# bryanlimy/CalciumGAN

Measured on AMD Instinct MI355X. Metric: training samples/sec (seq_len=2048, n_critic=5), higher is better.
Workload: dtype bf16; 1 GPU; cfg2: dichotomised-Gaussian sl2048 calcium signals, 102 neurons, batch 128/GPU, calciumgan num_units 64 k 24 s 2 m 10 layer_norm, wgan-gp n_critic 5 lambda 10, Keras Adam 1e-4; global_batch=128, seq_len=2048, parallelism=dp1, launch=hipGraph replay of train(), critic_layer1_on_interpolate=a*y_real + (1-a)*y_fake from the stored outputs (cg_lrelu_mix)

## Files before the change

### calciumgan_amd/csrc/dense_rows.hip

```cpp
#include "cg_common.h"

namespace {

constexpr int kDrThreads = 256;
constexpr int kDrPitch = 132;

struct DenseRowsArgs {
  const uint16_t* x;
  const uint16_t* w;
  const float* bias;
  float* y;
  long long rows;
  int Cx, N, Cy, epilogue;
};

template <int KSTEPS>
__global__ __launch_bounds__(kDrThreads, 2) void dense_rows_kernel(
    DenseRowsArgs a) {
  __shared__ float tile[4][16 * kDrPitch];
  const int lane = threadIdx.x & 63;
  const int wave = threadIdx.x >> 6;
  const int r16 = lane & 15;
  const int g = lane >> 4;
  act8 wf[KSTEPS][8];
// ... 1 lines not shown
  for (int ks = 0; ks < KSTEPS; ++ks)
#pragma unroll
    for (int nt = 0; nt < 8; ++nt)
      wf[ks][nt] = *reinterpret_cast<const act8*>(
          a.w + (((long long)(nt * 16 + r16) * KSTEPS + ks) * 16 + g) * 8);
  float* tl = tile[wave];
  const int tcol = (lane & 31) * 4;
  const int trow = lane >> 5;
  f32x4 bv = {0.f, 0.f, 0.f, 0.f};
  f32x4 keep = {0.f, 0.f, 0.f, 0.f};
#pragma unroll
  for (int e = 0; e < 4; ++e)
    if (tcol + e < a.N) {
      keep[e] = 1.f;
      if (a.bias) bv[e] = a.bias[tcol + e];
    }
  const bool sig = a.epilogue == CG_EPI_SIGMOID;

  const long long nblk = (a.rows + 15) / 16;
  const long long stride = (long long)gridDim.x * 4;
  long long blk = (long long)blockIdx.x * 4 + wave;
  auto load_a = [&](long long b, act8 (&dst)[KSTEPS]) {
    const long long row = b * 16 + r16;
    const bool ok = b < nblk && row < a.rows;
#pragma unroll
    for (int ks = 0; ks < KSTEPS; ++ks) {
      act8 v = {0, 0, 0, 0, 0, 0, 0, 0};
      if (ok)
        v = *reinterpret_cast<const act8*>(a.x + row * a.Cx + ks * 32 + g * 8);
      dst[ks] = v;
    }
  };
  auto compute = [&](long long b, const act8 (&af)[KSTEPS]) {
    f32x4 acc[8];
#pragma unroll
    for (int nt = 0; nt < 8; ++nt) acc[nt] = f32x4{0.f, 0.f, 0.f, 0.f};
#pragma unroll
    for (int ks = 0; ks < KSTEPS; ++ks)
#pragma unroll
      for (int nt = 0; nt < 8; ++nt)
        acc[nt] = cg_mfma_16x16x32(af[ks], wf[ks][nt],
                                                          acc[nt], 0, 0, 0);
#pragma unroll
    for (int nt = 0; nt < 8; ++nt)
#pragma unroll
      for (int r = 0; r < 4; ++r)
        tl[(4 * g + r) * kDrPitch + nt * 16 + r16] = acc[nt][r];
    __builtin_amdgcn_fence(__ATOMIC_RELEASE, "wavefront");
    __builtin_amdgcn_wave_barrier();
    __builtin_amdgcn_fence(__ATOMIC_ACQUIRE, "wavefront");
#pragma unroll 2
    for (int pass = 0; pass < 8; ++pass) {
      const int row = pass * 2 + trow;
      const long long m = b * 16 + row;
      f32x4 v = *reinterpret_cast<const f32x4*>(tl + row * kDrPitch + tcol);
#pragma unroll
      for (int e = 0; e < 4; ++e) {
        const float t = v[e] + bv[e];
        const float sg = 1.f / (1.f + __expf(-t));
        v[e] = keep[e] != 0.f ? (sig ? sg : t) : 0.f;
      }
      if (m < a.rows && tcol < a.Cy)
        *reinterpret_cast<f32x4*>(a.y + m * a.Cy + tcol) = v;
    }
    __builtin_amdgcn_fence(__ATOMIC_RELEASE, "wavefront");
    __builtin_amdgcn_wave_barrier();
    __builtin_amdgcn_fence(__ATOMIC_ACQUIRE, "wavefront");
  };
  act8 af0[KSTEPS], af1[KSTEPS];
  load_a(blk, af0);
  while (blk < nblk) {
    load_a(blk + stride, af1);
    compute(blk, af0);
    blk += stride;
    if (blk >= nblk) break;
    load_a(blk + stride, af0);
    compute(blk, af1);
    blk += stride;
  }
}


constexpr int kMaxInterp = 8;
struct DenseInterpArgs {
  const uint16_t* x;
  const uint16_t* w;
  const float* bias;
  const float* real;
  const float* alpha;
  uint16_t* x0[kMaxInterp];
  int n, B, L, Cx, N, Cr, Cp, epilogue;
};

template <int KSTEPS>
__global__ __launch_bounds__(kDrThreads, 2) void dense_rows_interp_kernel(
    DenseInterpArgs a) {
  __shared__ float tile[4][16 * kDrPitch];
  const int lane = threadIdx.x & 63;
  const int wave = threadIdx.x >> 6;
  const int r16 = lane & 15;
  const int g = lane >> 4;
  act8 wf[KSTEPS][8];
#pragma unroll
  for (int ks = 0; ks < KSTEPS; ++ks)
#pragma unroll
    for (int nt = 0; nt < 8; ++nt)
      wf[ks][nt] = *reinterpret_cast<const act8*>(
          a.w + (((long long)(nt * 16 + r16) * KSTEPS + ks) * 16 + g) * 8);
  float* tl = tile[wave];
  const int tcol = (lane & 31) * 4;
  const int trow = lane >> 5;
  f32x4 bv = {0.f, 0.f, 0.f, 0.f};
  f32x4 keep = {0.f, 0.f, 0.f, 0.f};
#pragma unroll
  for (int e = 0; e < 4; ++e)
    if (tcol + e < a.N) {
      keep[e] = 1.f;
      if (a.bias) bv[e] = a.bias[tcol + e];
    }
  const bool sig = a.epilogue == CG_EPI_SIGMOID;
  const long long R = (long long)a.B * a.L;
  const long long nblk = R / 16;
  const long long nitem = nblk * a.n;
  const long long stride = (long long)gridDim.x * 4;
  const long long seg = R * a.Cp;
  auto load_a = [&](long long blk, int k, bool ok, act8 (&dst)[KSTEPS]) {
    const long long row = (long long)k * R + blk * 16 + r16;
#pragma unroll
    for (int ks = 0; ks < KSTEPS; ++ks) {
      act8 v = {0, 0, 0, 0, 0, 0, 0, 0};
      if (ok) v = *reinterpret_cast<const act8*>(a.x + row * a.Cx + ks * 32 + g * 8);
      dst[ks] = v;
    }
  };
  auto store4 = [&](uint16_t* p, const f32x4& v) {
    *reinterpret_cast<uint2*>(p) = make_uint2(pack2act(v[0], v[1]), pack2act(v[2], v[3]));
  };
  auto compute = [&](long long blk, int k, const act8 (&af)[KSTEPS]) {
    f32x4 acc[8];
#pragma unroll
    for (int nt = 0; nt < 8; ++nt) acc[nt] = f32x4{0.f, 0.f, 0.f, 0.f};
#pragma unroll
    for (int ks = 0; ks < KSTEPS; ++ks)
#pragma unroll
      for (int nt = 0; nt < 8; ++nt)
        acc[nt] = cg_mfma_16x16x32(af[ks], wf[ks][nt], acc[nt], 0, 0, 0);
#pragma unroll
    for (int nt = 0; nt < 8; ++nt)
#pragma unroll
      for (int r = 0; r < 4; ++r)
        tl[(4 * g + r) * kDrPitch + nt * 16 + r16] = acc[nt][r];
    f32x4 rr[8];
#pragma unroll
    for (int pass = 0; pass < 8; ++pass) {
      const long long m = blk * 16 + pass * 2 + trow;
      const float* p = a.real + m * a.Cr + tcol;
      f32x4 v = {0.f, 0.f, 0.f, 0.f};
#pragma unroll
      for (int e = 0; e < 4; ++e)
        if (tcol + e < a.N) v[e] = p[e];
      rr[pass] = v;
    }
    __builtin_amdgcn_fence(__ATOMIC_RELEASE, "wavefront");
    __builtin_amdgcn_wave_barrier();
    __builtin_amdgcn_fence(__ATOMIC_ACQUIRE, "wavefront");
    const int b = (int)((blk * 16) / a.L);
    const float al = a.alpha ? a.alpha[k * a.B + b] : 0.f;
    uint16_t* x0 = a.x0[k];
#pragma unroll 2
    for (int pass = 0; pass < 8; ++pass) {
      const int row = pass * 2 + trow;
      const long long m = blk * 16 + row;
      f32x4 f = *reinterpret_cast<const f32x4*>(tl + row * kDrPitch + tcol);
      f32x4 xh;
#pragma unroll
      for (int e = 0; e < 4; ++e) {
        const float t = f[e] + bv[e];
        const float sg = 1.f / (1.f + __expf(-t));
        f[e] = keep[e] != 0.f ? (sig ? sg : t) : 0.f;
        xh[e] = al * rr[pass][e] + (1.f - al) * f[e];
      }
      if (tcol < a.Cp) {
        uint16_t* q = x0 + m * a.Cp + tcol;
        store4(q, rr[pass]);
        store4(q + seg, f);
        if (a.alpha) store4(q + 2 * seg, xh);
      }
    }
    __builtin_amdgcn_fence(__ATOMIC_RELEASE, "wavefront");
    __builtin_amdgcn_wave_barrier();
    __builtin_amdgcn_fence(__ATOMIC_ACQUIRE, "wavefront");
  };
  long long blk = (long long)blockIdx.x * 4 + wave;
  int k = 0;
  auto advance = [&](long long& bb, int& kk) {
    if (++kk == a.n) { kk = 0; bb += stride; }
  };
  act8 af0[KSTEPS], af1[KSTEPS];
  load_a(blk, k, blk < nblk, af0);
  (void)nitem;
  while (blk < nblk) {
    long long nb = blk; int nk = k;
    advance(nb, nk);
    load_a(nb, nk, nb < nblk, af1);
    compute(blk, k, af0);
    blk = nb; k = nk;
    if (blk >= nblk) break;
    advance(nb, nk);
    load_a(nb, nk, nb < nblk, af0);
    compute(blk, k, af1);
    blk = nb; k = nk;
  }
}

constexpr int kWideThreads = 256;
constexpr int kWideCols = 128;

struct DenseWideArgs {
  const uint16_t* x;
  const uint16_t* w;
  const float* bias;
  void* y;
  long long rows;
  int Cx, N, Cy, epilogue, out_act, panels;
  const float* real;
  const float* alpha;
  uint16_t* x0[kMaxInterp];
  long long seg_rows;
  int n_upd, L, Cr;
};

template <int KSTEPS>
__global__ __launch_bounds__(kWideThreads, KSTEPS <= 4 ? 2 : 1) void dense_rows_wide_kernel(
    DenseWideArgs a) {
  constexpr int kRowB = KSTEPS * 64 + 16;
  extern __shared__ __attribute__((aligned(16))) unsigned char wl[];
  const int tid = threadIdx.x;
  const int lane = tid & 63;
  const int wave = tid >> 6;
  const int r16 = lane & 15;
  const int g = lane >> 4;
  const int xcd = blockIdx.x & 7;
  const int j = blockIdx.x >> 3;
  const int panel = j % a.panels;
  const int rgroup = (j / a.panels) * 8 + xcd;
  const int ngroups = (int)(gridDim.x / 8 / a.panels) * 8;
  const int n0 = panel * kWideCols;
  for (int i = tid; i < kWideCols * KSTEPS * 4; i += kWideThreads) {
    const int c = i / (KSTEPS * 4);
    const int ks = (i / 4) % KSTEPS;
    const int gg = i & 3;
    const uint4 v = *reinterpret_cast<const uint4*>(
        a.w + (((long long)(n0 + c) * KSTEPS + ks) * 16 + gg) * 8);
    *reinterpret_cast<uint4*>(wl + c * kRowB + (ks * 4 + gg) * 16) = v;
  }
  __syncthreads();
  const int cq = (g & 1) * 16 + (g >> 1) * 8;
  float bv[4][8];
#pragma unroll
  for (int p = 0; p < 4; ++p)
#pragma unroll
    for (int e = 0; e < 8; ++e) {
      const int n = n0 + p * 32 + cq + e;
      bv[p][e] = (a.bias && n < a.N) ? a.bias[n] : 0.f;
    }
  const bool sig = a.epilogue == CG_EPI_SIGMOID;
  const int woff0 = r16 * kRowB + g * 16;

  const long long nblk = (a.rows + 31) / 32;
  const long long stride = (long long)ngroups * 4;
  long long blk = (long long)rgroup * 4 + wave;
  auto load_x = [&](long long b, act8 (&dst)[2][KSTEPS]) {
#pragma unroll
    for (int h = 0; h < 2; ++h) {
      long long row = b * 32 + h * 16 + r16;
      row = row < a.rows ? row : a.rows - 1;
      const uint16_t* src = a.x + row * a.Cx + g * 8;
#pragma unroll
      for (int ks = 0; ks < KSTEPS; ++ks)
        dst[h][ks] = *reinterpret_cast<const act8*>(src + ks * 32);
    }
  };
  auto compute = [&](long long b, const act8 (&xf)[2][KSTEPS]) {
    f32x4 acc[2][8];
#pragma unroll
    for (int h = 0; h < 2; ++h)
#pragma unroll
      for (int nt = 0; nt < 8; ++nt) acc[h][nt] = f32x4{0.f, 0.f, 0.f, 0.f};
    int woff = woff0;
    asm volatile("" : "+v"(woff));
    const unsigned char* wrow = wl + woff;
    act8 wa[8], wb[8];
// ... 31 lines not shown
    }
#pragma unroll
    for (int h = 0; h < 2; ++h) {
      const long long m = b * 32 + h * 16 + r16;
#pragma unroll
      for (int p = 0; p < 4; ++p) {
        float v[8];
#pragma unroll
        for (int r = 0; r < 4; ++r) {
          const auto sw = __builtin_amdgcn_permlane16_swap(
              __float_as_uint(acc[h][2 * p][r]),
              __float_as_uint(acc[h][2 * p + 1][r]), false, false);
          v[r] = __uint_as_float(sw[0]);
          v[4 + r] = __uint_as_float(sw[1]);
        }
        const int n = n0 + p * 32 + cq;
        if (m < a.rows && n < a.Cy) {
#pragma unroll
          for (int e = 0; e < 8; ++e) {
            const float t = v[e] + bv[p][e];
            const float sg = 1.f / (1.f + __expf(-t));
            v[e] = (n + e < a.N) ? (sig ? sg : t) : 0.f;
          }
          if (interp) {
            const long long rem = m - kupd * a.seg_rows;
            uint16_t* q = x0k + rem * a.Cy + n;
            const long long seg = a.seg_rows * a.Cy;
            *reinterpret_cast<uint4*>(q + seg) =
                make_uint4(pack2act(v[0], v[1]), pack2act(v[2], v[3]),
                           pack2act(v[4], v[5]), pack2act(v[6], v[7]));
            if (a.real) {
              const float* rp = a.real + rem * a.Cr + n;
              float rv[8], xh[8];
#pragma unroll
              for (int e = 0; e < 8; ++e) rv[e] = (n + e < a.N) ? rp[e] : 0.f;
              *reinterpret_cast<uint4*>(q) =
                  make_uint4(pack2act(rv[0], rv[1]), pack2act(rv[2], rv[3]),
                             pack2act(rv[4], rv[5]), pack2act(rv[6], rv[7]));
              if (a.alpha) {
                const float al =
                    a.alpha[kupd * (a.seg_rows / a.L) + (int)(rem / a.L)];
#pragma unroll
                for (int e = 0; e < 8; ++e) xh[e] = al * rv[e] + (1.f - al) * v[e];
                *reinterpret_cast<uint4*>(q + 2 * seg) =
                    make_uint4(pack2act(xh[0], xh[1]), pack2act(xh[2], xh[3]),
                               pack2act(xh[4], xh[5]), pack2act(xh[6], xh[7]));
              }
            }
          } else if (a.out_act) {
            *reinterpret_cast<uint4*>(reinterpret_cast<uint16_t*>(a.y) +
                                      m * a.Cy + n) =
                make_uint4(pack2act(v[0], v[1]), pack2act(v[2], v[3]),
                           pack2act(v[4], v[5]), pack2act(v[6], v[7]));
          } else {
            float* dst = reinterpret_cast<float*>(a.y) + m * a.Cy + n;
            *reinterpret_cast<f32x4*>(dst) = f32x4{v[0], v[1], v[2], v[3]};
            *reinterpret_cast<f32x4*>(dst + 4) = f32x4{v[4], v[5], v[6], v[7]};
          }
        }
      }
    }
  };
  act8 xf0[2][KSTEPS], xf1[2][KSTEPS];
  load_x(blk, xf0);
  while (blk < nblk) {
    load_x(blk + stride, xf1);
    compute(blk, xf0);
    blk += stride;
    if (blk >= nblk) break;
    load_x(blk + stride, xf0);
    compute(blk, xf1);
    blk += stride;
  }
}

template <int KSTEPS>
int launch_dense_wide(const DenseWideArgs& a, hipStream_t s) {
  const size_t lds = (size_t)kWideCols * (KSTEPS * 64 + 16);
  if (int e = cg_allow_dynamic_lds<&dense_rows_wide_kernel<KSTEPS>>(160 * 1024))
    return e;
  const int per_xcd = (KSTEPS <= 4 ? 64 : 32) / a.panels * a.panels;
  hipLaunchKernelGGL(dense_rows_wide_kernel<KSTEPS>, dim3(8 * per_xcd),
                     dim3(kWideThreads), lds, s, a);
  CG_LAUNCH_CHECK();
}

struct DenseWideInterp {
  const float* real;
  const float* alpha;
  void* const* x0;
  int n, B, L, Cr;
};

int dense_rows_wide(const void* x, const void* w, const float* bias, void* y,
                    long long rows, int Cx, int N, int Cy, int epilogue,
                    int out_act, hipStream_t s,
                    const DenseWideInterp* ip = nullptr) {
  if (Cx % 32 || N < 1 || Cy < N || Cy % 8) return CG_EINVAL;
  DenseWideArgs a;
  a.x = reinterpret_cast<const uint16_t*>(x);
  a.w = reinterpret_cast<const uint16_t*>(w);
  a.bias = bias;
  a.y = y;
  a.rows = rows;
  a.Cx = Cx; a.N = N; a.Cy = Cy; a.epilogue = epilogue; a.out_act = out_act;
  a.real = nullptr; a.alpha = nullptr; a.seg_rows = 1; a.n_upd = 0; a.L = 1; a.Cr = 0;
  for (int k = 0; k < kMaxInterp; ++k) a.x0[k] = nullptr;
  if (ip) {
    const long long seg = (long long)ip->B * ip->L;
    if (!ip->x0 || ip->n < 1 || ip->n > kMaxInterp || seg % 32 ||
        rows != seg * ip->n || (ip->real && ip->Cr < N) || (!ip->real && ip->alpha))
      return CG_EINVAL;
    a.real = ip->real; a.alpha = ip->alpha; a.seg_rows = seg;
    a.n_upd = ip->n; a.L = ip->L; a.Cr = ip->Cr;
    for (int k = 0; k < ip->n; ++k) {
      a.x0[k] = reinterpret_cast<uint16_t*>(ip->x0[k]);
      if (!a.x0[k]) return CG_EINVAL;
    }
  }
  a.panels = (N + kWideCols - 1) / kWideCols;
  if (a.panels > 32) return CG_EINVAL;
  switch (Cx / 32) {
    case 4: return launch_dense_wide<4>(a, s);
    case 8: return launch_dense_wide<8>(a, s);
    case 12: return launch_dense_wide<12>(a, s);
    case 16: return launch_dense_wide<16>(a, s);
    default: return CG_EINVAL;
  }
}

constexpr int kDwThreads = 256;
constexpr int kDwPitch = 144;

struct DenseWgradArgs {
  const uint16_t* x;
  const uint16_t* g;
  float* dw;
  long long rows, rows_per_split;
  int Cx, Cg, Cx_real, Cg_real, tiles_x, tiles_g;
  float* part;
};

__device__ __forceinline__ s16x4 dw_tr_read(const uint16_t* p) {
  return __builtin_amdgcn_ds_read_tr16_b64_v4i16(
      (__attribute__((address_space(3))) s16x4*)(p));
}
__device__ __forceinline__ act8 dw_join(s16x4 lo, s16x4 hi) {
  typedef __attribute__((ext_vector_type(8))) short s16x8;
  s16x8 v = {lo[0], lo[1], lo[2], lo[3], hi[0], hi[1], hi[2], hi[3]};
  return __builtin_bit_cast(act8, v);
}

__global__ __launch_bounds__(kDwThreads, 2) void dense_wgrad_kernel(
    DenseWgradArgs a) {
  __shared__ __attribute__((aligned(16))) uint16_t lx[2][32 * kDwPitch];
  __shared__ __attribute__((aligned(16))) uint16_t lg[2][32 * kDwPitch];
  const int tid = threadIdx.x;
  const int lane = tid & 63;
  const int wave = tid >> 6;
  const int r16 = lane & 15, g4 = lane >> 4, q = r16 >> 2, p = r16 & 3;
  const int wx = wave >> 1, wg = wave & 1;
  const int ntiles = a.tiles_x * a.tiles_g;
  const int xcd = blockIdx.x & 7;
  const int j = blockIdx.x >> 3;
  const int tile = j % ntiles;
  const long long split = (long long)(j / ntiles) * 8 + xcd;
// ... 129 lines not shown
  a.rows = rows;
  a.Cx = Cx; a.N = N; a.Cy = Cy; a.epilogue = epilogue;
  const long long nblk = (rows + 15) / 16;
  long long blocks = (nblk + 3) / 4;
  if (blocks > 512) blocks = 512;
  hipStream_t s = (hipStream_t)stream;
  dim3 grid((unsigned)blocks), block(kDrThreads);
  switch (Cx / 32) {
    case 1: hipLaunchKernelGGL(dense_rows_kernel<1>, grid, block, 0, s, a); break;
    case 2: hipLaunchKernelGGL(dense_rows_kernel<2>, grid, block, 0, s, a); break;
    case 3: hipLaunchKernelGGL(dense_rows_kernel<3>, grid, block, 0, s, a); break;
    default: hipLaunchKernelGGL(dense_rows_kernel<4>, grid, block, 0, s, a); break;
  }
  CG_LAUNCH_CHECK();
}

struct RealBcastArgs {
  const float* real;
  uint16_t* x0[kMaxInterp];
  long long total8;
  int n, N, Cr, Cp;
};
__global__ __launch_bounds__(256) void real_bcast_kernel(RealBcastArgs a) {
  const long long idx = (long long)blockIdx.x * 256 + threadIdx.x;
  if (idx >= a.total8) return;
  const int per_row = a.Cp / 8;
  const long long row = idx / per_row;
  const int c = (int)(idx - row * per_row) * 8;
  const float* rp = a.real + row * a.Cr + c;
  float v[8];
  if ((a.Cr & 3) == 0 && c + 8 <= a.N) {
    const f32x4 lo = *reinterpret_cast<const f32x4*>(rp);
    const f32x4 hi = *reinterpret_cast<const f32x4*>(rp + 4);
#pragma unroll
    for (int e = 0; e < 4; ++e) { v[e] = lo[e]; v[4 + e] = hi[e]; }
  } else {
#pragma unroll
    for (int e = 0; e < 8; ++e) v[e] = (c + e < a.N) ? rp[e] : 0.f;
  }
  const uint4 o = make_uint4(pack2act(v[0], v[1]), pack2act(v[2], v[3]),
                             pack2act(v[4], v[5]), pack2act(v[6], v[7]));
  for (int k = 0; k < a.n; ++k)
    *reinterpret_cast<uint4*>(a.x0[k] + row * a.Cp + c) = o;
}

extern "C" int cg_dense_rows_interp(const void* x, const void* w, const float* bias,
                                    const float* real, const float* alpha,
                                    void* const* x0, int n, int B, int L, int Cx,
                                    int N, int Cr, int Cp, int epilogue,
                                    void* stream) {
  if (!x || !w || !real || !x0 || n < 1 || n > kMaxInterp || B < 1 || L < 16 ||
      L % 16)
    return CG_EINVAL;
  if (epilogue != CG_EPI_NONE && epilogue != CG_EPI_SIGMOID) return CG_EINVAL;
  if (Cx > 128 || N > 128) {
    if (Cp < N || Cp % 8) return CG_EINVAL;
    const DenseWideInterp ip = {alpha ? real : nullptr, alpha, x0, n, B, L, Cr};
    const int rc = dense_rows_wide(x, w, bias, nullptr, (long long)n * B * L, Cx, N,
                                   Cp, epilogue, 0, (hipStream_t)stream, &ip);
    if (rc != 0 || alpha) return rc;
    RealBcastArgs ra;
    ra.real = real;
    for (int k = 0; k < kMaxInterp; ++k)
      ra.x0[k] = k < n ? reinterpret_cast<uint16_t*>(x0[k]) : nullptr;
    ra.total8 = (long long)B * L * (Cp / 8);
    ra.n = n; ra.N = N; ra.Cr = Cr; ra.Cp = Cp;
    hipLaunchKernelGGL(real_bcast_kernel,
                       dim3((unsigned)((ra.total8 + 255) / 256)), dim3(256), 0,
                       (hipStream_t)stream, ra);
    CG_LAUNCH_CHECK();
  }
  if (Cx % 32 || Cx < 32 || Cx > 128 || N < 1 || N > 128 || Cp != 128 || Cr < N)
    return CG_EINVAL;
  DenseInterpArgs a;
  a.x = reinterpret_cast<const uint16_t*>(x);
  a.w = reinterpret_cast<const uint16_t*>(w);
  a.bias = bias; a.real = real; a.alpha = alpha;
  for (int k = 0; k < kMaxInterp; ++k)
    a.x0[k] = k < n ? reinterpret_cast<uint16_t*>(x0[k]) : nullptr;
  for (int k = 0; k < n; ++k)
    if (!a.x0[k]) return CG_EINVAL;
  a.n = n; a.B = B; a.L = L; a.Cx = Cx; a.N = N; a.Cr = Cr; a.Cp = Cp;
  a.epilogue = epilogue;
  const long long nblk = (long long)B * L / 16;
  long long blocks = (nblk + 3) / 4;
  if (blocks > 512) blocks = 512;
  hipStream_t s = (hipStream_t)stream;
  dim3 grid((unsigned)blocks), block(kDrThreads);
  switch (Cx / 32) {
    case 1: hipLaunchKernelGGL(dense_rows_interp_kernel<1>, grid, block, 0, s, a); break;
    case 2: hipLaunchKernelGGL(dense_rows_interp_kernel<2>, grid, block, 0, s, a); break;
    case 3: hipLaunchKernelGGL(dense_rows_interp_kernel<3>, grid, block, 0, s, a); break;
    default: hipLaunchKernelGGL(dense_rows_interp_kernel<4>, grid, block, 0, s, a); break;
  }
  CG_LAUNCH_CHECK();
}

extern "C" int cg_dense_rows_act(const void* x, const void* w, void* y,
                                 long long rows, int Cx, int N, int Cy,
                                 void* stream) {
  if (!x || !w || !y || rows < 1) return CG_EINVAL;
  return dense_rows_wide(x, w, nullptr, y, rows, Cx, N, Cy, CG_EPI_NONE, 1,
                         (hipStream_t)stream);
}

extern "C" long long cg_dense_wgrad_ws_elems(long long rows, int Cx_real,
                                             int Cg_real);

namespace {
void dense_wgrad_split(long long rows, int ntiles, long long& nsplit,
                       long long& rps) {
  nsplit = (ntiles <= 4 ? 512 : 1024) / ntiles / 8 * 8;
  if (nsplit < 8) nsplit = 8;
  rps = (rows + nsplit - 1) / nsplit;
  rps = (rps + 31) / 32 * 32;
  nsplit = ((rows + rps - 1) / rps + 7) / 8 * 8;
}
}

extern "C" long long cg_dense_wgrad_ws_elems(long long rows, int Cx_real,
                                             int Cg_real) {
  if (rows < 1 || Cx_real < 1 || Cg_real < 1) return -1;
  const int ntiles = ((Cx_real + 127) / 128) * ((Cg_real + 127) / 128);
  long long nsplit, rps;
  dense_wgrad_split(rows, ntiles, nsplit, rps);
  return nsplit * (long long)Cx_real * Cg_real;
}

extern "C" int cg_dense_wgrad(const void* x, const void* g, float* dw,
                              long long rows, int Cx, int Cg, int Cx_real,
                              int Cg_real, float* ws, long long ws_elems,
                              void* stream) {
  if (!x || !g || !dw || rows < 1) return CG_EINVAL;
  if (Cx % 8 || Cg % 8 || Cx_real < 1 || Cg_real < 1 || Cx_real > Cx ||
      Cg_real > Cg)
    return CG_EINVAL;
  DenseWgradArgs a;
  a.x = reinterpret_cast<const uint16_t*>(x);
  a.g = reinterpret_cast<const uint16_t*>(g);
  a.dw = dw;
  a.rows = rows;
  a.Cx = Cx; a.Cg = Cg; a.Cx_real = Cx_real; a.Cg_real = Cg_real;
  a.tiles_x = (Cx_real + 127) / 128;
  a.tiles_g = (Cg_real + 127) / 128;
  const int ntiles = a.tiles_x * a.tiles_g;
  if (ntiles > 256) return CG_EINVAL;
  long long nsplit, rps;
  dense_wgrad_split(rows, ntiles, nsplit, rps);
  a.rows_per_split = rps;
  const long long n = (long long)Cx_real * Cg_real;
  if (ws && ws_elems < nsplit * n) return CG_EINVAL;
  a.part = ws;
  hipStream_t s = (hipStream_t)stream;
  hipLaunchKernelGGL(dense_wgrad_kernel, dim3((unsigned)(nsplit * ntiles)),
                     dim3(kDwThreads), 0, s, a);
  if (a.part)
    hipLaunchKernelGGL(dense_wgrad_reduce_kernel, dim3((unsigned)((n + 63) / 64)),
                       dim3(1024), 0, s, a.part, dw, n, (int)nsplit);
  CG_LAUNCH_CHECK();
}
```

### calciumgan_amd/csrc/pointwise.hip

```cpp
#include "cg_common.h"

namespace {

constexpr int kThreads = 256;

inline unsigned grid1d(long long work, int per_block, long long cap = 1 << 20) {
  long long b = (work + per_block - 1) / per_block;
  if (b < 1) b = 1;
  if (b > cap) b = cap;
  return (unsigned)b;
}

constexpr int kMaxParts = 2048;
constexpr long long kReduceWsElems = 4ll << 20;

struct FinishArgs {
  const float* ws;
  int nparts, ncol;
  long long pstride;
  int cstride;
  int nout;
  float* out[3];
  int cvalid[3];
  float scale;
// ... 1552 lines not shown
                         void* stream) {
  if (!dout || !y || !mean || !var || !gamma || !dy || !dgamma || !dbeta || !ws ||
      (act && !h) || Cp % 8 || Cp > 2048 || C > Cp || rows < 1)
    return CG_EINVAL;
  const int rpb = bn_rows_per_block(rows, Cp);
  const unsigned blocks = grid1d(rows, rpb, 1LL << 31);
  hipLaunchKernelGGL(bn_sums_kernel<1>, dim3(blocks), dim3(kThreads), 0,
                     cg_stream(stream), U16(y), U16(dout), U16(h), mean, var, rows, C, Cp,
                     rpb, eps, alpha, act, ws);
  FinishArgs f;
  f.ws = ws; f.nparts = (int)blocks; f.ncol = Cp; f.pstride = 2ll * Cp;
  f.cstride = Cp; f.nout = 2; f.scale = 1.f;
  f.out[0] = dbeta; f.out[1] = dgamma; f.out[2] = nullptr;
  f.cvalid[0] = f.cvalid[1] = C; f.cvalid[2] = 0;
  launch_finish(f, cg_stream(stream));
  const long long total8 = rows * Cp / 8;
  hipLaunchKernelGGL(bn_bwd_apply_kernel,
                     dim3(grid1d(total8, kThreads, 1LL << 31)), dim3(kThreads), 0,
                     cg_stream(stream), U16(dout), U16(h), U16(y), mean, var, gamma,
                     dgamma, dbeta, U16W(dy), C, Cp, eps, alpha, act,
                     1.f / (float)rows, total8);
  CG_LAUNCH_CHECK();
}

extern "C" int cg_dense1_fwd(const void* h, const float* w, const float* bias,
                             float* out, int nB, int Lt, int C, int Cp,
                             void* stream) {
  const int F = Lt * Cp;
  if (Cp % 8 || C > Cp || nB < 1) return CG_EINVAL;
  if (F >= 8192)
    hipLaunchKernelGGL(dense1_fwd_kernel<1024>, dim3(nB), dim3(1024), 0,
                       cg_stream(stream), U16(h), w, bias, out, F, C, Cp,
                       (const float*)nullptr, (uint16_t*)nullptr, 1, 1.f);
  else
    hipLaunchKernelGGL(dense1_fwd_kernel<256>, dim3(nB), dim3(256), 0, cg_stream(stream),
                       U16(h), w, bias, out, F, C, Cp, (const float*)nullptr,
                       (uint16_t*)nullptr, 1, 1.f);
  CG_LAUNCH_CHECK();
}

extern "C" int cg_dense1_fwd_bwd(const void* h, const float* w, const float* bias,
                                 float* out, const float* coef, void* delta,
                                 int nB, int Lt, int C, int Cp, int seg_size,
                                 float alpha, void* stream) {
  const int F = Lt * Cp;
  if (Cp % 8 || C > Cp || nB < 1 || seg_size < 1 || !coef || !delta)
    return CG_EINVAL;
  if (F >= 8192)
    hipLaunchKernelGGL(dense1_fwd_kernel<1024>, dim3(nB), dim3(1024), 0,
                       cg_stream(stream), U16(h), w, bias, out, F, C, Cp, coef,
                       U16W(delta), seg_size, alpha);
  else
    hipLaunchKernelGGL(dense1_fwd_kernel<256>, dim3(nB), dim3(256), 0, cg_stream(stream),
                       U16(h), w, bias, out, F, C, Cp, coef, U16W(delta), seg_size,
                       alpha);
  CG_LAUNCH_CHECK();
}

__global__ void gp_critic_loss_kernel(float* __restrict__ norm, float* __restrict__ gp,
                                      float* __restrict__ coef,
                                      const float* __restrict__ d_out,
                                      float* __restrict__ loss, int B, float scale,
                                      int squared, float coef_mul) {
  gp_tail<true>([=](int b) { return gp_load_norm(norm, b, squared); }, gp, coef,
                d_out, loss, B, scale, coef_mul);
}

extern "C" int cg_gp_critic_loss(float* norm, float* gp, float* coef,
                                 const float* d_out, float* loss, int B,
                                 float penalty, int squared, float coef_mul,
                                 void* stream) {
  if (!norm || !gp || !coef || !d_out || !loss || B < 1) return CG_EINVAL;
  hipLaunchKernelGGL(gp_critic_loss_kernel, dim3(1), dim3(kThreads), 0, cg_stream(stream),
                     norm, gp, coef, d_out, loss, B, penalty, squared, coef_mul);
  CG_LAUNCH_CHECK();
}

__device__ __forceinline__ float slot_sum(const float* __restrict__ ws, int P, int b) {
  float s = 0.f;
  for (int j = 0; j < P; ++j) s += ws[(long long)b * P + j];
  return s;
}

__global__ __launch_bounds__(kThreads) void gp_loss_scale_kernel(
    const float* __restrict__ ssq_ws, int P, float* __restrict__ norm,
    float* __restrict__ gp, float* __restrict__ coef,
    const float* __restrict__ d_out, float* __restrict__ loss, int B, float scale,
    float coef_mul, const uint16_t* __restrict__ g, uint16_t* __restrict__ dst,
    long long n, long long total8) {
  if (blockIdx.x + 1 == gridDim.x) {
    gp_tail<true>(
        [=](int b) {
          const float nv = sqrtf(slot_sum(ssq_ws, P, b));
          norm[b] = nv;
          return nv;
        },
        gp, coef, d_out, loss, B, scale, coef_mul);
    return;
  }
  const long long idx = (long long)blockIdx.x * kThreads + threadIdx.x;
  if (idx >= total8) return;
  const long long i = idx * 8;
  const int b = (int)(i / n);
  const float c = gp_coef(sqrtf(slot_sum(ssq_ws, P, b)), B, scale, coef_mul);
  float v[8], o[8];
  load8(g + i, v);
#pragma unroll
  for (int e = 0; e < 8; ++e) o[e] = c * v[e];
  store8(dst + i, o);
}

extern "C" int cg_gp_loss_scale(const float* ssq_ws, int P, float* norm, float* gp,
                                float* coef, const float* d_out, float* loss,
                                int B, float penalty, float coef_mul,
                                const void* g, void* dst, long long n,
                                void* stream) {
  if (!ssq_ws || P < 1 || !norm || !gp || !coef || !d_out || !loss || B < 1)
    return CG_EINVAL;
  if ((g != nullptr) != (dst != nullptr) || (g && (n < 8 || n % 8))) return CG_EINVAL;
  const long long total8 = g ? (long long)B * n / 8 : 0;
  const unsigned blocks = (unsigned)((total8 + kThreads - 1) / kThreads) + 1;
  hipLaunchKernelGGL(gp_loss_scale_kernel, dim3(blocks), dim3(kThreads), 0,
                     cg_stream(stream), ssq_ws, P, norm, gp, coef, d_out, loss, B,
                     penalty, coef_mul, U16(g), U16W(dst), n, total8);
  CG_LAUNCH_CHECK();
}

extern "C" int cg_dense1_bwd(const float* w, const float* coef, const void* h,
                             void* delta, int nB, int Lt, int C, int Cp,
                             int seg_size, float alpha, void* stream) {
  const int F = Lt * Cp;
  if (Cp % 8 || C > Cp || nB < 1 || seg_size < 1) return CG_EINVAL;
  const long long total8 = (long long)nB * F / 8;
  hipLaunchKernelGGL(dense1_bwd_kernel, dim3(grid1d(total8, kThreads, 1LL << 31)),
                     dim3(kThreads), 0, cg_stream(stream), w, coef, U16(h),
                     U16W(delta), F, C, Cp, seg_size, alpha, total8);
  CG_LAUNCH_CHECK();
}

extern "C" int cg_dense1_wgrad(const void* x, const float* coef,
                               const float* bias_coef, float* dw, float* db,
                               int nB, int Lt, int C, int Cp, int seg_size,
                               float* ws, void* stream) {
  const int F = Lt * Cp;
  if (Cp % 8 || C > Cp || nB < 1 || seg_size < 1) return CG_EINVAL;
  const int gx = (F / 8 + kThreads - 1) / kThreads;
  int gy = 512 / gx;
  if (gy < 1) gy = 1;
  if (gy > nB) gy = nB;
  const int Fpad = gx * kThreads * 8;
  if (ws && (long long)gy * Fpad + gy > kReduceWsElems) return CG_EINVAL;
  hipLaunchKernelGGL(dense1_wgrad_kernel, dim3(gx, gy), dim3(kThreads), 0,
                     cg_stream(stream), U16(x), coef, bias_coef, dw, db, nB, F, C,
                     Cp, seg_size, ws, Fpad);
  if (ws)
    hipLaunchKernelGGL(dense1_wgrad_finish, dim3((F + kThreads - 1) / kThreads),
                       dim3(kThreads), 0, cg_stream(stream), ws, dw, db, gy, F, Fpad, C,
                       Cp, bias_coef ? 1 : 0);
  CG_LAUNCH_CHECK();
}

constexpr int kBceLdsGroups = 4096;

extern "C" int cg_dense1_bce(const void* h, const float* w, const float* bias,
                             float* out, float* coef_d, float* coef_g,
                             void* delta_d, void* delta_g, float* loss,
                             const float* scale_d, const float* scale_g, int B,
                             int Lt, int C, int Cp, float alpha, float* ws,
                             void* stream) {
  const int F = Lt * Cp;
  if (Cp % 8 || C > Cp || B < 1 || !h || !w || !bias || !out || !loss)
    return CG_EINVAL;
  if (delta_g && !delta_d) return CG_EINVAL;
  if (ws && 3ll * B > kReduceWsElems) return CG_EINVAL;
  const dim3 grid(2 * B);
  const bool lds = delta_d && F / 8 <= kBceLdsGroups;
#define CG_BCE_LAUNCH(NT, ROW)                                                      \
  hipLaunchKernelGGL((dense1_bce_kernel<NT, ROW>), grid, dim3(NT), 0,               \
                     cg_stream(stream), U16(h), w, bias, out, coef_d, coef_g,       \
                     U16W(delta_d), U16W(delta_g), scale_d, scale_g, ws, loss, B,   \
                     F, C, Cp, alpha)
  if (F >= 8192) {
    if (lds) CG_BCE_LAUNCH(1024, kBceLdsGroups);
    else CG_BCE_LAUNCH(1024, 1);
  } else {
    if (lds) CG_BCE_LAUNCH(256, 1024);
    else CG_BCE_LAUNCH(256, 1);
  }
#undef CG_BCE_LAUNCH
  if (ws)
    hipLaunchKernelGGL(dense1_bce_finish, dim3(1), dim3(kThreads), 0, cg_stream(stream),
                       ws, loss, B);
  CG_LAUNCH_CHECK();
}

extern "C" int cg_unshuffle_mask(const void* e, const void* h, void* delta,
                                 const int* shifts, int nB, int w, int Cp,
                                 int seg_size, float alpha, void* stream) {
  if (Cp % 8 || nB < 1 || w < 1 || seg_size < 1) return CG_EINVAL;
  const long long total8 = (long long)nB * w * Cp / 8;
  hipLaunchKernelGGL(unshuffle_mask_kernel,
                     dim3(grid1d(total8, kThreads, 1LL << 31)), dim3(kThreads),
                     0, cg_stream(stream), U16(e), U16(h), U16W(delta), shifts, w, Cp,
                     seg_size, alpha, total8);
  CG_LAUNCH_CHECK();
}

// ... 227 lines not shown
```

### calciumgan_amd/csrc/wgrad.hip

```cpp
#include "cg_common.h"

#include <string.h>

#include <map>
#include <mutex>
#include <vector>

namespace {

#ifndef CG_WGRAD_SHIFT
#define CG_WGRAD_SHIFT 96
#endif
#ifdef CG_WGRAD_TRACE
constexpr int kWTraceParts = 5;
__device__ unsigned g_wgrad_trace[256 * 8 * kWTraceParts];
#define CG_WTR_PARAMS , unsigned (&wtr)[kWTraceParts], unsigned& wtt
#define CG_WTR_ARGS , wtr, wtt
#define CG_WTR(acc, t, part) do { unsigned long long n_; \
    asm volatile("s_memtime %0\n\ts_waitcnt lgkmcnt(0)" : "=s"(n_)::"memory"); \
    (acc)[part] += (unsigned)n_ - (t); (t) = (unsigned)n_; } while (0)
#define CG_WTR_BEGIN unsigned wtr[kWTraceParts] = {}; unsigned wtt; \
  do { unsigned long long n_; \
    asm volatile("s_memtime %0\n\ts_waitcnt lgkmcnt(0)" : "=s"(n_)::"memory"); \
    wtt = (unsigned)n_; } while (0)
// ... 873 lines not shown
  const int rot = 0;
#else
  const int rot = ((int)blockIdx.x >> 6) % m.n;
#endif
  CG_WTR_BEGIN;
  for (int k = 0; k < m.n; ++k) {
    int li = k + rot;
    if (li >= m.n) li -= m.n;
    const int gz = m.gz[li];
    int bx, by, bz;
    const int cnt = m.cnt[li];
    int id = (int)blockIdx.x - m.lo[li];
    const bool mine = id >= 0 && id < cnt;
#ifndef CG_WGRAD_NO_SHIFT
    id += (li * CG_WGRAD_SHIFT) % cnt;
    if (id >= cnt) id -= cnt;
#endif
    if (mine && wgrad_block(m.a[li], m.zcnt[li], id, bx, by, bz)) {
      bz += m.zofs[li];
      if (m.tt[li] == 128)
        wgrad_body<R, TPW, false, true, 128, ALLT>(m.a[li], bx, by, bz, gz, -1, -1, 1 CG_WTR_ARGS);
      else
        wgrad_body<R, TPW, false, true, 64, ALLT>(m.a[li], bx, by, bz, gz, -1, -1, 1 CG_WTR_ARGS);
    }
    CG_WTR(wtr, wtt, 3);
    __syncthreads();
    CG_WTR(wtr, wtt, 4);
  }
  CG_WTR_END;
}

constexpr int kFlexMaxItems = 8;
constexpr int kFlexItemInts = 6;

struct WgradFlex {
  int n;
  int tt[kMaxBatch];
  int cw[kMaxBatch];
  const int* table;
  WgradArgs a[kMaxBatch];
};

template <int R, int TPW, int ALLT>
__global__ __launch_bounds__(512) void wgrad_flex_kernel(WgradFlex m) {
  CG_WTR_BEGIN;
  const int* it = m.table + (size_t)blockIdx.x * (kFlexMaxItems * kFlexItemInts);
  for (int k = 0; k < kFlexMaxItems; ++k, it += kFlexItemInts) {
    const int li = __builtin_amdgcn_readfirstlane(it[0]);
    if (li < 0) break;
    const int bx = __builtin_amdgcn_readfirstlane(it[1]);
    const int by = __builtin_amdgcn_readfirstlane(it[2]);
    const int k0 = __builtin_amdgcn_readfirstlane(it[3]);
    const int kn = __builtin_amdgcn_readfirstlane(it[4]);
    const int ps = __builtin_amdgcn_readfirstlane(it[5]);
    if (m.tt[li] == 128)
      wgrad_body<R, TPW, false, true, 128, ALLT>(m.a[li], bx, by, k0, 1, kn, ps, m.cw[li] CG_WTR_ARGS);
    else
      wgrad_body<R, TPW, false, true, 64, ALLT>(m.a[li], bx, by, k0, 1, kn, ps, m.cw[li] CG_WTR_ARGS);
    CG_WTR(wtr, wtt, 3);
    __syncthreads();
    CG_WTR(wtr, wtt, 4);
  }
  CG_WTR_END;
}

struct FlexReduceItem {
  const float* part;
  float* dw;
  const int* tiles;
  int gx, gy, tpw, taps, Cx_real, Cg_real;
  int store, zc;
  int cw;
  const float* bias_part;
  float* dbias;
};
struct FlexReduceArgs {
  int n;
  FlexReduceItem it[kMaxBatch];
};

__global__ __launch_bounds__(256) void wgrad_flex_reduce_kernel(FlexReduceArgs ra) {
  const FlexReduceItem& it = ra.it[blockIdx.y];
  __shared__ f32x4 red[256];
  if (it.bias_part && blockIdx.x == 0) {
    for (int c = threadIdx.x; c < it.gy * 64; c += 256) {
      float s = 0.f;
      for (int bx = 0; bx < it.cw; ++bx) {
        const int t = (c >> 6) * it.gx + bx;
        const int p0 = it.tiles[2 * t], cnt = it.tiles[2 * t + 1];
        for (int z = 0; z < cnt; ++z) s += it.bias_part[(long long)(p0 + z) * 64 + (c & 63)];
      }
      if (c < it.Cg_real) {
        if (it.store) it.dbias[c] = s;
        else it.dbias[c] += s;
      }
    }
  }
  const int per_tile = it.tpw * 8 * 512;
  const long long total = (long long)it.gx * it.gy * per_tile;
  const int zc = it.zc;
  const int epb = 256 / zc;
  const int el = (int)threadIdx.x % epb;
  const int zi = (int)threadIdx.x / epb;
  for (long long base = (long long)blockIdx.x * epb; base < total;
       base += (long long)gridDim.x * epb) {
    const long long e = base + el;
    const int tile = (int)(base / per_tile);
    const int rem = (int)(e - (long long)tile * per_tile);
    const int p0 = it.tiles[2 * tile], cnt = it.tiles[2 * tile + 1];
    const int chunk = (cnt + zc - 1) / zc;
    const int z0 = zi * chunk;
    const int z1 = z0 + chunk < cnt ? z0 + chunk : cnt;
    const float* p = it.part + ((long long)p0 * per_tile + rem) * 4;
    const long long stride = (long long)per_tile * 4;
    const f32x4 sum = reduce_splits(p, true, z0, z1, stride, zc, zi, el, epb, red);
    if (zi != 0) continue;
    reduce_commit(it, sum, rem, tile % it.gx, tile / it.gx);
  }
}

inline int ilog2(int v) {
  int l = 0;
  while ((1 << l) < v) ++l;
  return l;
}

inline unsigned wgrad_grid(const WgradArgs& a, int gz) {
  if (a.gmode == 3) return (unsigned)(a.pgx * a.pgy * gz);
  const int per_split = a.pgx * a.pgy / a.gsz;
  const int groups = per_split * gz;
  return (unsigned)((groups + 7) / 8 * 8 * a.gsz);
}

template <int R, int TPW, bool ROWSPLIT, bool PIPE, int TT, int ALLT = 0>
int launch_wgrad1(const WgradArgs& a, dim3 grid, size_t lds, hipStream_t s) {
  if (int e = cg_allow_dynamic_lds<&wgrad_kernel<R, TPW, ROWSPLIT, PIPE, TT, ALLT>>(
          160 * 1024))
    return e;
  CG_LAUNCH_PROF(CG_FAMILY_WGRAD, (wgrad_kernel<R, TPW, ROWSPLIT, PIPE, TT, ALLT>),
                 dim3(wgrad_grid(a, grid.z)), dim3(512), lds, s, a, (int)grid.z);
  CG_LAUNCH_CHECK();
}

template <int R, int TPW, bool ROWSPLIT>
int launch_wgrad(const WgradArgs& a, dim3 grid, size_t lds, bool pipe, int tt,
                 hipStream_t s) {
  constexpr int T0 = ROWSPLIT ? 256 : 64;
  const bool allt = !ROWSPLIT && pipe && a.taps == 8 * TPW && a.nseg == 1;
  if constexpr (R == 2 && TPW == 3 && !ROWSPLIT) {
    if (a.ring && allt) {
      if (tt == 128)
        return launch_wgrad1<R, TPW, ROWSPLIT, true, 128, 2>(a, grid, 2 * lds, s);
      return launch_wgrad1<R, TPW, ROWSPLIT, true, 64, 2>(a, grid, 2 * lds, s);
    }
  }
  if (!ROWSPLIT && tt == 128) {
    if (allt)
      return launch_wgrad1<R, TPW, ROWSPLIT, true, ROWSPLIT ? 256 : 128,
                           !ROWSPLIT>(a, grid, 2 * lds, s);
    return launch_wgrad1<R, TPW, ROWSPLIT, true, ROWSPLIT ? 256 : 128>(
        a, grid, 2 * lds, s);
  }
  if (pipe && allt)
    return launch_wgrad1<R, TPW, ROWSPLIT, true, T0, !ROWSPLIT>(a, grid, 2 * lds,
                                                                s);
  if (pipe) return launch_wgrad1<R, TPW, ROWSPLIT, true, T0>(a, grid, 2 * lds, s);
  return launch_wgrad1<R, TPW, ROWSPLIT, false, T0>(a, grid, lds, s);
}

}

namespace {

// ... 716 lines not shown
```

Measured before the change: 11260 samples/s.

## Stage real rows in LDS, split interp kernel, per-block gp coef, parallel bias reduce

The interpolate dense kernel is templated on whether alpha is present. When k==0 it loads each block's real rows once with coalesced vector loads into LDS, so the other interpolation copies read them from LDS instead of re-reading global memory with strided scalar loads. In the non-xhat path the real copy is written to all x0 slots once rather than per k. The gp loss scale kernel computes the per-sample coefficient once per block through shared memory. The bias reduction in the flex wgrad reduce is spread across blocks with unrolled loads. Together these cut redundant global traffic, at the cost of extra LDS and code paths.

```diff
diff --git a/calciumgan_amd/csrc/dense_rows.hip b/calciumgan_amd/csrc/dense_rows.hip
--- a/calciumgan_amd/csrc/dense_rows.hip
+++ b/calciumgan_amd/csrc/dense_rows.hip
@@ -107,6 +107,7 @@
 
 
 constexpr int kMaxInterp = 8;
+constexpr int kRealVecs = 7;
 struct DenseInterpArgs {
   const uint16_t* x;
   const uint16_t* w;
@@ -115,12 +116,14 @@
   const float* alpha;
   uint16_t* x0[kMaxInterp];
   int n, B, L, Cx, N, Cr, Cp, epilogue;
+  int run;
 };
 
-template <int KSTEPS>
+template <int KSTEPS, bool XHAT>
 __global__ __launch_bounds__(kDrThreads, 2) void dense_rows_interp_kernel(
     DenseInterpArgs a) {
   __shared__ float tile[4][16 * kDrPitch];
+  extern __shared__ __attribute__((aligned(16))) float real_lds[];
   const int lane = threadIdx.x & 63;
   const int wave = threadIdx.x >> 6;
   const int r16 = lane & 15;
@@ -133,6 +136,7 @@
       wf[ks][nt] = *reinterpret_cast<const act8*>(
           a.w + (((long long)(nt * 16 + r16) * KSTEPS + ks) * 16 + g) * 8);
   float* tl = tile[wave];
+  float* rl = real_lds + wave * kRealVecs * 256;
   const int tcol = (lane & 31) * 4;
   const int trow = lane >> 5;
   f32x4 bv = {0.f, 0.f, 0.f, 0.f};
@@ -146,75 +150,131 @@
   const bool sig = a.epilogue == CG_EPI_SIGMOID;
   const long long R = (long long)a.B * a.L;
   const long long nblk = R / 16;
-  const long long nitem = nblk * a.n;
   const long long stride = (long long)gridDim.x * 4;
   const long long seg = R * a.Cp;
-  auto load_a = [&](long long blk, int k, bool ok, act8 (&dst)[KSTEPS]) {
-    const long long row = (long long)k * R + blk * 16 + r16;
-#pragma unroll
-    for (int ks = 0; ks < KSTEPS; ++ks) {
-      act8 v = {0, 0, 0, 0, 0, 0, 0, 0};
-      if (ok) v = *reinterpret_cast<const act8*>(a.x + row * a.Cx + ks * 32 + g * 8);
-      dst[ks] = v;
-    }
-  };
-  auto store4 = [&](uint16_t* p, const f32x4& v) {
-    *reinterpret_cast<uint2*>(p) = make_uint2(pack2act(v[0], v[1]), pack2act(v[2], v[3]));
-  };
-  auto compute = [&](long long blk, int k, const act8 (&af)[KSTEPS]) {
-    f32x4 acc[8];
-#pragma unroll
-    for (int nt = 0; nt < 8; ++nt) acc[nt] = f32x4{0.f, 0.f, 0.f, 0.f};
+  auto load_a = [&](long long blk, int k, act8 (&dst)[KSTEPS]) {
+    const long long bc = blk < nblk ? blk : nblk - 1;
+    const long long row = (long long)k * R + bc * 16 + r16;
 #pragma unroll
     for (int ks = 0; ks < KSTEPS; ++ks)
-#pragma unroll
-      for (int nt = 0; nt < 8; ++nt)
-        acc[nt] = cg_mfma_16x16x32(af[ks], wf[ks][nt], acc[nt], 0, 0, 0);
-#pragma unroll
-    for (int nt = 0; nt < 8; ++nt)
-#pragma unroll
-      for (int r = 0; r < 4; ++r)
-        tl[(4 * g + r) * kDrPitch + nt * 16 + r16] = acc[nt][r];
-    f32x4 rr[8];
-#pragma unroll
-    for (int pass = 0; pass < 8; ++pass) {
-      const long long m = blk * 16 + pass * 2 + trow;
-      const float* p = a.real + m * a.Cr + tcol;
-      f32x4 v = {0.f, 0.f, 0.f, 0.f};
-#pragma unroll
-      for (int e = 0; e < 4; ++e)
-        if (tcol + e < a.N) v[e] = p[e];
-      rr[pass] = v;
-    }
+      dst[ks] = *reinterpret_cast<const act8*>(a.x + row * a.Cx + ks * 32 + g * 8);
+  };
+  const int nvec = 4 * a.Cr;
+  f32x4 rq[kRealVecs];
+  auto fetch_real = [&](long long blk, int j0, int j1) {
+    const f32x4* src = reinterpret_cast<const f32x4*>(a.real + blk * 16 * a.Cr);
+#pragma unroll
+    for (int j = j0; j < j1; ++j) {
+      const int i = j * 64 + lane;
+      rq[j] = src[i < nvec ? i : nvec - 1];
+    }
+  };
+  auto stash_real = [&](int j0, int j1) {
+#pragma unroll
+    for (int j = j0; j < j1; ++j) {
+      const int i = j * 64 + lane;
+      if (i < nvec) reinterpret_cast<f32x4*>(rl)[i] = rq[j];
+    }
+  };
+  auto wave_sync = [&]() {
     __builtin_amdgcn_fence(__ATOMIC_RELEASE, "wavefront");
     __builtin_amdgcn_wave_barrier();
     __builtin_amdgcn_fence(__ATOMIC_ACQUIRE, "wavefront");
-    const int b = (int)((blk * 16) / a.L);
-    const float al = a.alpha ? a.alpha[k * a.B + b] : 0.f;
+  };
+  auto real4 = [&](int row, long long m) {
+    f32x4 rr = {0.f, 0.f, 0.f, 0.f};
+    if (a.run) {
+#pragma unroll
+      for (int e = 0; e < 4; ++e)
+        if (tcol + e < a.N) rr[e] = rl[row * a.Cr + tcol + e];
+    } else {
+#pragma unroll
+      for (int e = 0; e < 4; ++e)
+        if (tcol + e < a.N) rr[e] = a.real[m * a.Cr + tcol + e];
+    }
+    return rr;
+  };
+  auto store4 = [&](uint16_t* p, const f32x4& v) {
+    *reinterpret_cast<uint2*>(p) = make_uint2(pack2act(v[0], v[1]), pack2act(v[2], v[3]));
+  };
+  auto compute = [&](long long blk, int k, const act8 (&af)[KSTEPS]) {
+    f32x4 acc[8];
+#pragma unroll
+    for (int nt = 0; nt < 8; ++nt) acc[nt] = f32x4{0.f, 0.f, 0.f, 0.f};
+#pragma unroll
+    for (int ks = 0; ks < KSTEPS; ++ks)
+#pragma unroll
+      for (int nt = 0; nt < 8; ++nt)
+        acc[nt] = cg_mfma_16x16x32(af[ks], wf[ks][nt], acc[nt], 0, 0, 0);
+#pragma unroll
+    for (int nt = 0; nt < 8; ++nt)
+#pragma unroll
+      for (int r = 0; r < 4; ++r)
+        tl[(4 * g + r) * kDrPitch + nt * 16 + r16] = acc[nt][r];
+    const bool fetch = k == 0 && a.run;
+    if (XHAT) {
+      if (fetch) {
+        fetch_real(blk, 0, 4);
+        stash_real(0, 4);
+        fetch_real(blk, 4, kRealVecs);
+        stash_real(4, kRealVecs);
+      }
+    } else if (fetch) {
+      fetch_real(blk, 0, kRealVecs);
+    }
+    wave_sync();
     uint16_t* x0 = a.x0[k];
-#pragma unroll 2
-    for (int pass = 0; pass < 8; ++pass) {
-      const int row = pass * 2 + trow;
-      const long long m = blk * 16 + row;
+    auto fake4 = [&](int row) {
       f32x4 f = *reinterpret_cast<const f32x4*>(tl + row * kDrPitch + tcol);
-      f32x4 xh;
 #pragma unroll
       for (int e = 0; e < 4; ++e) {
         const float t = f[e] + bv[e];
         const float sg = 1.f / (1.f + __expf(-t));
         f[e] = keep[e] != 0.f ? (sig ? sg : t) : 0.f;
-        xh[e] = al * rr[pass][e] + (1.f - al) * f[e];
       }
-      if (tcol < a.Cp) {
+      return f;
+    };
+    if (XHAT) {
+      const int b = (int)((blk * 16) / a.L);
+      const float al = a.alpha[k * a.B + b];
+#pragma unroll 2
+      for (int pass = 0; pass < 8; ++pass) {
+        const int row = pass * 2 + trow;
+        const long long m = blk * 16 + row;
+        const f32x4 f = fake4(row);
+        const f32x4 rr = real4(row, m);
+        f32x4 xh;
+#pragma unroll
+        for (int e = 0; e < 4; ++e) xh[e] = __builtin_fmaf(al, rr[e], (1.f - al) * f[e]);
         uint16_t* q = x0 + m * a.Cp + tcol;
-        store4(q, rr[pass]);
+        store4(q, rr);
         store4(q + seg, f);
-        if (a.alpha) store4(q + 2 * seg, xh);
+        store4(q + 2 * seg, xh);
       }
-    }
-    __builtin_amdgcn_fence(__ATOMIC_RELEASE, "wavefront");
-    __builtin_amdgcn_wave_barrier();
-    __builtin_amdgcn_fence(__ATOMIC_ACQUIRE, "wavefront");
+    } else {
+#pragma unroll 2
+      for (int pass = 0; pass < 8; ++pass) {
+        const int row = pass * 2 + trow;
+        const long long m = blk * 16 + row;
+        store4(x0 + m * a.Cp + tcol + seg, fake4(row));
+      }
+      if (k == 0) {
+        if (fetch) {
+          stash_real(0, kRealVecs);
+          wave_sync();
+        }
+#pragma unroll 2
+        for (int pass = 0; pass < 8; ++pass) {
+          const int row = pass * 2 + trow;
+          const long long m = blk * 16 + row;
+          const f32x4 rr = real4(row, m);
+          const uint2 rb = make_uint2(pack2act(rr[0], rr[1]), pack2act(rr[2], rr[3]));
+          for (int kk = 0; kk < a.n; ++kk)
+            *reinterpret_cast<uint2*>(a.x0[kk] + m * a.Cp + tcol) = rb;
+        }
+      }
+    }
+    wave_sync();
   };
   long long blk = (long long)blockIdx.x * 4 + wave;
   int k = 0;
@@ -222,17 +282,16 @@
     if (++kk == a.n) { kk = 0; bb += stride; }
   };
   act8 af0[KSTEPS], af1[KSTEPS];
-  load_a(blk, k, blk < nblk, af0);
-  (void)nitem;
+  load_a(blk, k, af0);
   while (blk < nblk) {
     long long nb = blk; int nk = k;
     advance(nb, nk);
-    load_a(nb, nk, nb < nblk, af1);
+    load_a(nb, nk, af1);
     compute(blk, k, af0);
     blk = nb; k = nk;
     if (blk >= nblk) break;
     advance(nb, nk);
-    load_a(nb, nk, nb < nblk, af0);
+    load_a(nb, nk, af0);
     compute(blk, k, af1);
     blk = nb; k = nk;
   }
@@ -430,6 +489,17 @@
   const int per_xcd = (KSTEPS <= 4 ? 64 : 32) / a.panels * a.panels;
   hipLaunchKernelGGL(dense_rows_wide_kernel<KSTEPS>, dim3(8 * per_xcd),
                      dim3(kWideThreads), lds, s, a);
+  CG_LAUNCH_CHECK();
+}
+
+static_assert(4 * 16 * kDrPitch * 4 + 4 * kRealVecs * 1024 <= 64 * 1024, "LDS");
+template <int KSTEPS>
+int launch_dense_interp(const DenseInterpArgs& a, dim3 grid, dim3 block, hipStream_t s) {
+  const size_t lds = a.run ? (size_t)4 * kRealVecs * 1024 : 0;
+  if (a.alpha)
+    hipLaunchKernelGGL((dense_rows_interp_kernel<KSTEPS, true>), grid, block, lds, s, a);
+  else
+    hipLaunchKernelGGL((dense_rows_interp_kernel<KSTEPS, false>), grid, block, lds, s, a);
   CG_LAUNCH_CHECK();
 }
 
@@ -725,18 +795,18 @@
     if (!a.x0[k]) return CG_EINVAL;
   a.n = n; a.B = B; a.L = L; a.Cx = Cx; a.N = N; a.Cr = Cr; a.Cp = Cp;
   a.epilogue = epilogue;
+  a.run = 64 * Cr <= kRealVecs * 1024 && reinterpret_cast<uintptr_t>(real) % 16 == 0;
   const long long nblk = (long long)B * L / 16;
   long long blocks = (nblk + 3) / 4;
   if (blocks > 512) blocks = 512;
   hipStream_t s = (hipStream_t)stream;
   dim3 grid((unsigned)blocks), block(kDrThreads);
   switch (Cx / 32) {
-    case 1: hipLaunchKernelGGL(dense_rows_interp_kernel<1>, grid, block, 0, s, a); break;
-    case 2: hipLaunchKernelGGL(dense_rows_interp_kernel<2>, grid, block, 0, s, a); break;
-    case 3: hipLaunchKernelGGL(dense_rows_interp_kernel<3>, grid, block, 0, s, a); break;
-    default: hipLaunchKernelGGL(dense_rows_interp_kernel<4>, grid, block, 0, s, a); break;
-  }
-  CG_LAUNCH_CHECK();
+    case 1: return launch_dense_interp<1>(a, grid, block, s);
+    case 2: return launch_dense_interp<2>(a, grid, block, s);
+    case 3: return launch_dense_interp<3>(a, grid, block, s);
+    default: return launch_dense_interp<4>(a, grid, block, s);
+  }
 }
 
 extern "C" int cg_dense_rows_act(const void* x, const void* w, void* y,
diff --git a/calciumgan_amd/csrc/pointwise.hip b/calciumgan_amd/csrc/pointwise.hip
--- a/calciumgan_amd/csrc/pointwise.hip
+++ b/calciumgan_amd/csrc/pointwise.hip
@@ -1658,6 +1658,7 @@
   return s;
 }
 
+template <bool kPerBlock>
 __global__ __launch_bounds__(kThreads) void gp_loss_scale_kernel(
     const float* __restrict__ ssq_ws, int P, float* __restrict__ norm,
     float* __restrict__ gp, float* __restrict__ coef,
@@ -1677,10 +1678,22 @@
   const long long idx = (long long)blockIdx.x * kThreads + threadIdx.x;
   if (idx >= total8) return;
   const long long i = idx * 8;
-  const int b = (int)(i / n);
-  const float c = gp_coef(sqrtf(slot_sum(ssq_ws, P, b)), B, scale, coef_mul);
   float v[8], o[8];
-  load8(g + i, v);
+  float c;
+  if constexpr (kPerBlock) {
+    __shared__ float slot[kThreads];
+    load8(g + i, v);
+    const int b = (int)((long long)blockIdx.x * (kThreads * 8) / n);
+    if ((int)threadIdx.x < P) slot[threadIdx.x] = ssq_ws[(long long)b * P + threadIdx.x];
+    __syncthreads();
+    float s = 0.f;
+    for (int j = 0; j < P; ++j) s += slot[j];
+    c = gp_coef(sqrtf(s), B, scale, coef_mul);
+  } else {
+    const int b = (int)(i / n);
+    c = gp_coef(sqrtf(slot_sum(ssq_ws, P, b)), B, scale, coef_mul);
+    load8(g + i, v);
+  }
 #pragma unroll
   for (int e = 0; e < 8; ++e) o[e] = c * v[e];
   store8(dst + i, o);
@@ -1696,9 +1709,14 @@
   if ((g != nullptr) != (dst != nullptr) || (g && (n < 8 || n % 8))) return CG_EINVAL;
   const long long total8 = g ? (long long)B * n / 8 : 0;
   const unsigned blocks = (unsigned)((total8 + kThreads - 1) / kThreads) + 1;
-  hipLaunchKernelGGL(gp_loss_scale_kernel, dim3(blocks), dim3(kThreads), 0,
-                     cg_stream(stream), ssq_ws, P, norm, gp, coef, d_out, loss, B,
-                     penalty, coef_mul, U16(g), U16W(dst), n, total8);
+  if (g && n % (8 * kThreads) == 0 && P <= kThreads)
+    hipLaunchKernelGGL(gp_loss_scale_kernel<true>, dim3(blocks), dim3(kThreads), 0,
+                       cg_stream(stream), ssq_ws, P, norm, gp, coef, d_out, loss, B,
+                       penalty, coef_mul, U16(g), U16W(dst), n, total8);
+  else
+    hipLaunchKernelGGL(gp_loss_scale_kernel<false>, dim3(blocks), dim3(kThreads), 0,
+                       cg_stream(stream), ssq_ws, P, norm, gp, coef, d_out, loss, B,
+                       penalty, coef_mul, U16(g), U16W(dst), n, total8);
   CG_LAUNCH_CHECK();
 }
 
diff --git a/calciumgan_amd/csrc/wgrad.hip b/calciumgan_amd/csrc/wgrad.hip
--- a/calciumgan_amd/csrc/wgrad.hip
+++ b/calciumgan_amd/csrc/wgrad.hip
@@ -979,13 +979,23 @@
 __global__ __launch_bounds__(256) void wgrad_flex_reduce_kernel(FlexReduceArgs ra) {
   const FlexReduceItem& it = ra.it[blockIdx.y];
   __shared__ f32x4 red[256];
-  if (it.bias_part && blockIdx.x == 0) {
-    for (int c = threadIdx.x; c < it.gy * 64; c += 256) {
+  if (it.bias_part && threadIdx.x < 64) {
+    for (int cb = blockIdx.x; cb < it.gy; cb += gridDim.x) {
+      const int c = cb * 64 + (int)threadIdx.x;
       float s = 0.f;
       for (int bx = 0; bx < it.cw; ++bx) {
-        const int t = (c >> 6) * it.gx + bx;
+        const int t = cb * it.gx + bx;
         const int p0 = it.tiles[2 * t], cnt = it.tiles[2 * t + 1];
-        for (int z = 0; z < cnt; ++z) s += it.bias_part[(long long)(p0 + z) * 64 + (c & 63)];
+        const float* bp = it.bias_part + (long long)p0 * 64 + threadIdx.x;
+        int z = 0;
+        for (; z + 8 <= cnt; z += 8) {
+          float v[8];
+#pragma unroll
+          for (int j = 0; j < 8; ++j) v[j] = bp[(long long)(z + j) * 64];
+#pragma unroll
+          for (int j = 0; j < 8; ++j) s += v[j];
+        }
+        for (; z < cnt; ++z) s += bp[(long long)z * 64];
       }
       if (c < it.Cg_real) {
         if (it.store) it.dbias[c] = s;
```

Measured after the change: 11340 samples/s, median of 6. About the same (+0.7%).
